# luigifcruz/radio-core

Hardware: AMD Instinct MI355X
Metric: IQ Msamples/s through Tuner+WBFM at 1024 channels (higher is better)
Workload: dtype f32

## Files before the change

### radio-core_amd/csrc/fft_kernel.h

```cpp
#pragma once

#include <hip/hip_runtime.h>

#include <cstdio>
#include <cstdlib>
#include <type_traits>

#include "fft_engine.h"
#include "tile_ns.h"

namespace rcfm {
RCFM_NS_OPEN
namespace fftk {

constexpr int W = RCFM_TILE_W;
constexpr int kLogW = W == 16 ? 4 : W == 8 ? 3 : 2;
static_assert((1 << kLogW) == W, "tile width: 4, 8 or 16 lines");
constexpr int kThreads = 256 * W / 16;

__device__ __forceinline__ float2 cmul(float2 a, float2 b) {
    typedef float v2f __attribute__((ext_vector_type(2)));
    v2f A, B, D;
    A.x = a.x; A.y = a.y; B.x = b.x; B.y = b.y;
    asm("v_pk_mul_f32 %0, %1, %2 op_sel:[0,0] op_sel_hi:[0,1]" : "=v"(D) : "v"(A), "v"(B));
// ... 72 lines not shown
    x0 = cadd(x0, cadd(a, b));
    x1 = cadd_mi(t1, u1);
    x4 = cadd_pi(t1, u1);
    x2 = cadd_mi(t2, u2);
    x3 = cadd_pi(t2, u2);
}

__device__ __forceinline__ void dft7(float2& x0, float2& x1, float2& x2, float2& x3, float2& x4, float2& x5, float2& x6) {
    constexpr float c1 = 0.62348980185873353053f, c2 = -0.22252093395631440429f, c3 = -0.90096886790241912624f;
    constexpr float s1 = 0.78183148246802980871f, s2 = 0.97492791218182360702f, s3 = 0.43388373911755812048f;
    const float2 a1 = cadd(x1, x6), a2 = cadd(x2, x5), a3 = cadd(x3, x4);
    const float2 b1 = csub(x1, x6), b2 = csub(x2, x5), b3 = csub(x3, x4);
    const float2 t1 = make_float2(x0.x + c1 * a1.x + c2 * a2.x + c3 * a3.x, x0.y + c1 * a1.y + c2 * a2.y + c3 * a3.y);
    const float2 t2 = make_float2(x0.x + c2 * a1.x + c3 * a2.x + c1 * a3.x, x0.y + c2 * a1.y + c3 * a2.y + c1 * a3.y);
    const float2 t3 = make_float2(x0.x + c3 * a1.x + c1 * a2.x + c2 * a3.x, x0.y + c3 * a1.y + c1 * a2.y + c2 * a3.y);
    const float2 u1 = make_float2(s1 * b1.x + s2 * b2.x + s3 * b3.x, s1 * b1.y + s2 * b2.y + s3 * b3.y);
    const float2 u2 = make_float2(s2 * b1.x - s3 * b2.x - s1 * b3.x, s2 * b1.y - s3 * b2.y - s1 * b3.y);
    const float2 u3 = make_float2(s3 * b1.x - s1 * b2.x + s2 * b3.x, s3 * b1.y - s1 * b2.y + s2 * b3.y);
    x0 = cadd(x0, cadd(a1, cadd(a2, a3)));
    x1 = cadd_mi(t1, u1);
    x6 = cadd_pi(t1, u1);
    x2 = cadd_mi(t2, u2);
    x5 = cadd_pi(t2, u2);
    x3 = cadd_mi(t3, u3);
    x4 = cadd_pi(t3, u3);
}

template <int R>
__device__ __forceinline__ void dft_nat(float2* v) {
    if constexpr (R == 2) {
        dft2(v[0], v[1]);
    } else if constexpr (R == 3) {
        dft3(v[0], v[1], v[2]);
    } else if constexpr (R == 4) {
        dft4(v[0], v[1], v[2], v[3]);
    } else if constexpr (R == 5) {
        dft5(v[0], v[1], v[2], v[3], v[4]);
    } else if constexpr (R == 7) {
        dft7(v[0], v[1], v[2], v[3], v[4], v[5], v[6]);
    } else {
        constexpr int Ra = (R % 7 == 0) ? 7 : (R % 5 == 0) ? 5 : (R % 4 == 0) ? 4 : (R % 3 == 0) ? 3 : 2;
        constexpr int Rb = R / Ra;
        static_assert(Ra * Rb == R && Rb > 1, "radix must be 2-3-5-7 smooth");
        float2 y[R];
#pragma unroll
        for (int n2 = 0; n2 < Rb; ++n2) {
            float2 t[Ra];
#pragma unroll
            for (int n1 = 0; n1 < Ra; ++n1) t[n1] = v[Rb * n1 + n2];
            dft_nat<Ra>(t);
#pragma unroll
            for (int k1 = 0; k1 < Ra; ++k1) {
                const int m = (n2 * k1) % R;
                if (m == 0) {
                    y[k1 * Rb + n2] = t[k1];
                } else {
                    const double a = -6.28318530717958647692 * (double)m / (double)R;
                    y[k1 * Rb + n2] = cmul(t[k1], make_float2((float)__builtin_cos(a), (float)__builtin_sin(a)));
                }
            }
        }
#pragma unroll
        for (int k1 = 0; k1 < Ra; ++k1) {
            dft_nat<Rb>(&y[k1 * Rb]);
#pragma unroll
            for (int k2 = 0; k2 < Rb; ++k2) v[k1 + Ra * k2] = y[k1 * Rb + k2];
        }
    }
}


__device__ __forceinline__ void dft6(float2* v) {
    dft3(v[0], v[2], v[4]);
    dft3(v[1], v[3], v[5]);
    v[3] = cmul(v[3], make_float2(0.5f, -0.86602540378443864676f));
    v[5] = cmul(v[5], make_float2(-0.5f, -0.86602540378443864676f));
    dft2(v[0], v[1]);
    dft2(v[2], v[3]);
    dft2(v[4], v[5]);
    const float2 y0 = v[0], y3 = v[1], y1 = v[2], y4 = v[3], y2 = v[4], y5 = v[5];
    v[0] = y0; v[1] = y1; v[2] = y2; v[3] = y3; v[4] = y4; v[5] = y5;
}

__device__ __forceinline__ void dft8(float2* v) {
    constexpr float h = 0.70710678118654752440f;
    dft4(v[0], v[2], v[4], v[6]);
    dft4(v[1], v[3], v[5], v[7]);
    v[3] = cmul(v[3], make_float2(h, -h));
    v[5] = mul_mi(v[5]);
    v[7] = cmul(v[7], make_float2(-h, -h));
    dft2(v[0], v[1]);
    dft2(v[2], v[3]);
    dft2(v[4], v[5]);
    dft2(v[6], v[7]);
    const float2 y0 = v[0], y4 = v[1], y1 = v[2], y5 = v[3], y2 = v[4], y6 = v[5], y3 = v[6], y7 = v[7];
    v[0] = y0; v[1] = y1; v[2] = y2; v[3] = y3; v[4] = y4; v[5] = y5; v[6] = y6; v[7] = y7;
}

__device__ __forceinline__ void dft10(float2* v) {
    dft5(v[0], v[2], v[4], v[6], v[8]);
    dft5(v[1], v[3], v[5], v[7], v[9]);
    v[3] = cmul(v[3], make_float2(0.80901699437494742410f, -0.58778525229247312917f));
    v[5] = cmul(v[5], make_float2(0.30901699437494742410f, -0.95105651629515357212f));
    v[7] = cmul(v[7], make_float2(-0.30901699437494742410f, -0.95105651629515357212f));
    v[9] = cmul(v[9], make_float2(-0.80901699437494742410f, -0.58778525229247312917f));
    dft2(v[0], v[1]);
    dft2(v[2], v[3]);
    dft2(v[4], v[5]);
    dft2(v[6], v[7]);
    dft2(v[8], v[9]);
    const float2 y0 = v[0], y5 = v[1], y1 = v[2], y6 = v[3], y2 = v[4], y7 = v[5], y3 = v[6], y8 = v[7],
                 y4 = v[8], y9 = v[9];
    v[0] = y0; v[1] = y1; v[2] = y2; v[3] = y3; v[4] = y4;
    v[5] = y5; v[6] = y6; v[7] = y7; v[8] = y8; v[9] = y9;
}

template <int R>
__device__ __forceinline__ void dif_stage(float2* tile, const float2* tw, int L, int mt, int swz) {
    const int m = mt / R;
    const int step = L / mt;
    const int nb = (L / R) * W;
    for (int e = threadIdx.x; e < nb; e += kThreads) {
        const int w = e & (W - 1);
        const int b = e / W;
        const int g = b / m;
        const int kp = b - g * m;
        const int base = g * mt + kp;
        float2 v[R];
#pragma unroll
        for (int q = 0; q < R; ++q) {
            const int row = base + q * m;
            v[q] = tile[row * W + (w ^ (swz & row & (W - 1)))];
        }
        if constexpr (R == 2) dft2(v[0], v[1]);
        if constexpr (R == 3) dft3(v[0], v[1], v[2]);
        if constexpr (R == 4) dft4(v[0], v[1], v[2], v[3]);
        if constexpr (R == 5) dft5(v[0], v[1], v[2], v[3], v[4]);
        if constexpr (R == 6) dft6(v);
        if constexpr (R == 7) dft7(v[0], v[1], v[2], v[3], v[4], v[5], v[6]);
        if constexpr (R == 8) dft8(v);
        if constexpr (R == 10) dft10(v);
        if constexpr (R > 10) dft_nat<R>(v);
        const int tstep = kp * step;
#pragma unroll
        for (int q = 1; q < R; ++q) v[q] = cmul(v[q], tw[q * tstep]);
#pragma unroll
        for (int q = 0; q < R; ++q) {
            const int row = base + q * m;
            tile[row * W + (w ^ (swz & row & (W - 1)))] = v[q];
        }
    }
}

__device__ __forceinline__ float2 big_twiddle(const FftPassDev& d, unsigned e) {
    const float2 c = d.coarse[e >> d.fine_bits];
    const float th = d.fine_step * (float)(e & ((1u << d.fine_bits) - 1u));
    const float t2 = th * th;
    const float s = th * (1.f - t2 * (1.f / 6.f) * (1.f - t2 * (1.f / 20.f)));
    const float co = 1.f - t2 * 0.5f * (1.f - t2 * (1.f / 12.f) * (1.f - t2 * (1.f / 30.f)));
    return cmul(c, make_float2(co, -s));
}

struct LineId {
    int batch;
    int64_t o1, o2, i;
};

template <class T, class = void>
struct fetch_count { static constexpr int value = 1; };
template <class T>
struct fetch_count<T, std::void_t<decltype(T::kFetches)>> { static constexpr int value = T::kFetches; };

template <class T, class = void>
struct has_ctx : std::false_type {};
template <class T>
struct has_ctx<T, std::void_t<decltype(T::kCtx)>> : std::true_type {};

template <class LoadOp>
__device__ __forceinline__ float2 load_now(const LoadOp& load, const LineId& id, int l, int64_t base, unsigned off) {
    if constexpr (fetch_count<LoadOp>::value == 3)
        return load.post(id, l, load.fetch(id, l, base, off), load.fetch2(id, l, base, off),
                         load.fetch3(id, l, base, off));
    else if constexpr (fetch_count<LoadOp>::value == 2)
        return load.post(id, l, load.fetch(id, l, base, off), load.fetch2(id, l, base, off));
    else if constexpr (has_ctx<LoadOp>::value)
        return load.post(id, l, load.fetch(id, l, base, off), load.prepare(id));
    else
        return load.post(id, l, load.fetch(id, l, base, off));
}

template <class T, class = void>
struct has_half_zones : std::false_type {};
template <class T>
struct has_half_zones<T, std::void_t<decltype(T::kHalfZones)>> : std::bool_constant<T::kHalfZones> {};

template <class T, class = void>
struct has_aux : std::false_type {};
template <class T>
struct has_aux<T, std::void_t<decltype(T::kAux)>> : std::true_type {};

template <class StoreOp>
__device__ __forceinline__ void store_now(const StoreOp& store, const LineId& id, int k, int64_t base, unsigned off,
                                          float2 v) {
    if constexpr (has_aux<StoreOp>::value) store(id, k, base, off, v, store.fetch_aux(id, k, base, off));
    else store(id, k, base, off, v);
}

template <class LoadOp, class StoreOp>
__global__ __launch_bounds__(kThreads) void k_fft_pass(FftPassDev d, LoadOp load, StoreOp store) {
    extern __shared__ __attribute__((aligned(16))) unsigned char smem_raw[];
    const FftPass& p = d.p;
    const int L = p.L;
    float2* tile = reinterpret_cast<float2*>(smem_raw);
    float2* tw = tile + L * W;
    uint16_t* pos = reinterpret_cast<uint16_t*>(tw + L);

    const int tid = threadIdx.x;
    const int64_t tiles_inner = (p.n_inner + W - 1) / W;
    int64_t t = blockIdx.x;
    const int64_t ti = t % tiles_inner;
    t /= tiles_inner;
    LineId id;
    id.batch = blockIdx.y;
    id.o2 = t % p.n_o2;
    id.o1 = t / p.n_o2;
    const int64_t i0 = ti * W;
    const int wvalid = (int)((p.n_inner - i0) < W ? (p.n_inner - i0) : W);
    const int64_t in_base = (int64_t)id.batch * d.in_batch + id.o1 * p.in_o1 + id.o2 * p.in_o2 +
                            (p.in_t ? (i0 >> 4) * p.in_t + (i0 & 15) : i0 * p.in_i);
    const int64_t out_base = (int64_t)id.batch * d.out_batch + id.o1 * p.out_o1 + id.o2 * p.out_o2 +
                             (p.out_t ? (i0 >> 4) * p.out_t + (i0 & 15) : i0 * p.out_i);
    const int swz = p.load_along_l ? (W - 1) : 0;

    for (int e = tid; e < L; e += kThreads) {
        tw[e] = d.stage_tw[e];
        pos[e] = d.pos[e];
    }
    if (p.load_along_l) {
        for (int e = tid; e < L * W; e += kThreads) {
            const int w = e / L, l = e - w * L;
            float2 v = make_float2(0.f, 0.f);
            if (w < wvalid) {
                id.i = i0 + w;
                v = load_now(load, id, l, in_base, (unsigned)(w * p.in_i + l));
            }
            tile[l * W + (w ^ (l & (W - 1)))] = v;
        }
    } else {
        for (int e = tid; e < L * W; e += kThreads) {
            const int l = e / W, w = e & (W - 1);
            float2 v = make_float2(0.f, 0.f);
            if (w < wvalid) {
                id.i = i0 + w;
                v = load_now(load, id, l, in_base, (unsigned)(l * p.in_l + w * p.in_i));
            }
            tile[l * W + w] = v;
        }
    }
    __syncthreads();

    int mt = L;
    for (int s = 0; s < p.nstages; ++s) {
        const int r = p.radix[s];
        switch (r) {
            case 2: dif_stage<2>(tile, tw, L, mt, swz); break;
            case 3: dif_stage<3>(tile, tw, L, mt, swz); break;
            case 4: dif_stage<4>(tile, tw, L, mt, swz); break;
            case 5: dif_stage<5>(tile, tw, L, mt, swz); break;
            case 6: dif_stage<6>(tile, tw, L, mt, swz); break;
            case 7: dif_stage<7>(tile, tw, L, mt, swz); break;
            case 8: dif_stage<8>(tile, tw, L, mt, swz); break;
            case 12: dif_stage<12>(tile, tw, L, mt, swz); break;
            case 15: dif_stage<15>(tile, tw, L, mt, swz); break;
            case 16: dif_stage<16>(tile, tw, L, mt, swz); break;
            case 20: dif_stage<20>(tile, tw, L, mt, swz); break;
            case 24: dif_stage<24>(tile, tw, L, mt, swz); break;
            case 25: dif_stage<25>(tile, tw, L, mt, swz); break;
            case 32: dif_stage<32>(tile, tw, L, mt, swz); break;
            default: dif_stage<10>(tile, tw, L, mt, swz); break;
        }
        mt /= r;
        __syncthreads();
    }

    const unsigned tw_base = (unsigned)(id.o1 * p.tw_o1 + id.o2 * p.tw_o2 + i0 * p.tw_i);
    for (int e = tid; e < L * W; e += kThreads) {
        const int k = e / W, w = e & (W - 1);
        if (w >= wvalid) continue;
        const int row = pos[k];
        float2 v = tile[row * W + (w ^ (swz & row & (W - 1)))];
        if (p.has_twiddle) v = cmul(v, big_twiddle(d, (tw_base + (unsigned)w * (unsigned)p.tw_i) * (unsigned)k));
        id.i = i0 + w;
        store_now(store, id, k, out_base, (unsigned)(k * p.out_k + w * p.out_i), v);
    }
}


constexpr unsigned kXcdGroupMax = 15;
struct BlockPos {
    unsigned tile, batch;
};
struct VBlock {
    unsigned x, y, z, gx, gy, gz;
};
__device__ __forceinline__ VBlock vblock_hw() {
    return VBlock{blockIdx.x, blockIdx.y, blockIdx.z, gridDim.x, gridDim.y, gridDim.z};
}
__device__ __forceinline__ BlockPos block_pos(const VBlock& vb);
__device__ __forceinline__ BlockPos block_pos() { return block_pos(vblock_hw()); }
__device__ __forceinline__ BlockPos block_pos(const VBlock& vb) {
    const unsigned gx = vb.gx, x = vb.x, z = vb.z;
    if (gx <= kXcdGroupMax) {
        if (vb.gy == 1 && (z | 7u) < vb.gz) {
// ... 550 lines not shown
    const bool has1 = c0 + 1 < count;
    const int c1 = has1 ? c0 + 1 : c0;
    const int i0 = (int)bp.tile * W;
    const int left = (int)p1.n_inner - i0;
    const int wvalid = left < W ? left : W;
    const int64_t in_base = (int64_t)id.batch * d1.in_batch + (int64_t)i0 * p1.in_i;
    const int blk16 = mid.blk16;
    const int64_t mid_tile = blk16 ? (int64_t)(i0 >> 4) * blk16 + (i0 & 15) : (int64_t)i0;
    const int64_t mid_base0 = (int64_t)c0 * (blk16 ? mid.stride : d1.out_batch) + mid_tile;
    const int64_t mid_base1 = (int64_t)c1 * (blk16 ? mid.stride : d1.out_batch) + mid_tile;
    const int64_t out_base0 = (int64_t)c0 * d2.out_batch + i0;
    const int64_t out_base1 = (int64_t)c1 * d2.out_batch + i0;
    const unsigned in_i = (unsigned)p1.in_i, mid_k = blk16 ? 16u : (unsigned)p1.out_k, out_k = (unsigned)p2.out_k;
    const int wc = w < wvalid ? w : 0;

    auto lane_off = [&](int it) -> unsigned {
        int g = rg + RG * it;
        if (rowsL % RG != 0) g = g < rowsL ? g : 0;
        return (unsigned)last_stage_base<L, R0, R1, RL, S>(g) * mid_k + (unsigned)wc;
    };
    auto q_off = [&](int q) -> int64_t { return (int64_t)((L / RL) * q) * mid_k; };

    float2 v[nld];
#pragma unroll
    for (int it = 0; it < nld; ++it) {
        int e = tid + T * it;
        if ((L * W) % T != 0) e = e < L * W ? e : 0;
        const int wl = e / L, l = e - wl * L;
        const int wcl = wl < wvalid ? wl : 0;
        id.i = i0 + wcl;
        v[it] = load.fetch(id, l, in_base, (unsigned)wcl * in_i + (unsigned)l);
    }
    for (int e = tid; e < L; e += T) tw[e] = d1.stage_tw[e];
#pragma unroll
    for (int it = 0; it < nld; ++it) {
        const int e = tid + T * it;
        const int wl = e / L, l = e - wl * L;
        id.i = i0 + wl;
        const float2 x = load.post(id, l, v[it]);
        if ((L * W) % T == 0 || e < L * W) tile[lds_slot<true>(l, wl)] = x;
    }
    lds_barrier();
    stage_lds<L, R0, L, true, RG>(tile, tw, w, rg);
    lds_barrier();
    if constexpr (S >= 3) {
        stage_lds<L, R1, L / R0, true, RG>(tile, tw, w, rg);
        lds_barrier();
    }
    if constexpr (S >= 4) {
        stage_lds<L, R2, L / (R0 * R1), true, RG>(tile, tw, w, rg);
        lds_barrier();
    }

    using In0 = decltype(mid.fetch0(mid_base0, mid_base1, 0u));
    In0 a0[nitL * RL];
#pragma unroll
    for (int it = 0; it < nitL; ++it)
#pragma unroll
        for (int q = 0; q < RL; ++q)
            a0[it * RL + q] = mid.fetch0(mid_base0 + q_off(q), mid_base1 + q_off(q), lane_off(it));

    id.i = i0 + w;
    using Keep = typename MidOp::Keep;
    float2 u0[nitL * RL];
    Keep keep[nitL * RL];
#pragma unroll
    for (int it = 0; it < nitL; ++it) {
        const int g = rg + RG * it;
        if ((rowsL % RG == 0) || g < rowsL) {
            float2 x[RL];
#pragma unroll
            for (int q = 0; q < RL; ++q) x[q] = tile[lds_slot<true>(g * RL + q, w)];
            dft_p<RL>(x);
#pragma unroll
            for (int q = 0; q < RL; ++q)
                u0[it * RL + q] = mid.first(x[dft_slot<RL>(q)], a0[it * RL + q], keep[it * RL + q]);
        }
        __builtin_amdgcn_sched_barrier(0);
    }
    lds_barrier();
#pragma unroll
    for (int it = 0; it < nitL; ++it) {
        const int g = rg + RG * it;
        if ((rowsL % RG == 0) || g < rowsL) {
            const int kb = last_stage_base<L, R0, R1, RL, S>(g);
#pragma unroll
            for (int q = 0; q < RL; ++q) tile[lds_slot<true>(kb + (L / RL) * q, w)] = u0[it * RL + q];
        }
    }
    lds_barrier();

    const unsigned f = (unsigned)((int64_t)(i0 + w) * p2.tw_i);
    const float2 D = big_twiddle(d2, f * (unsigned)(L / RL));
    const bool lane_ok = w < wvalid;
    auto second_transform = [&](int64_t out_base) {
        stage_lds<L, R0, L, true, RG>(tile, tw, w, rg);
        lds_barrier();
        if constexpr (S >= 3) {
            stage_lds<L, R1, L / R0, true, RG>(tile, tw, w, rg);
            lds_barrier();
        }
        if constexpr (S >= 4) {
            stage_lds<L, R2, L / (R0 * R1), true, RG>(tile, tw, w, rg);
            lds_barrier();
        }
#pragma unroll
        for (int it = 0; it < nitL; ++it) {
            const int g = rg + RG * it;
            if ((rowsL % RG == 0) || g < rowsL) {
                float2 x[RL];
#pragma unroll
                for (int q = 0; q < RL; ++q) x[q] = tile[lds_slot<true>(g * RL + q, w)];
                dft_p<RL>(x);
                const int kb = last_stage_base<L, R0, R1, RL, S>(g);
                float2 Tw = big_twiddle(d2, f * (unsigned)kb);
                if (lane_ok) {
#pragma unroll
                    for (int q = 0; q < RL; ++q) {
                        const int k = kb + (L / RL) * q;
                        const float2 y = cmul(x[dft_slot<RL>(q)], Tw);
                        Tw = cmul(Tw, D);
                        store(id, k, out_base, (unsigned)k * out_k + (unsigned)w, y);
                    }
                }
            }
        }
    };

    float a1[nitL * RL];
#pragma unroll
    for (int it = 0; it < nitL; ++it)
#pragma unroll
        for (int q = 0; q < RL; ++q) a1[it * RL + q] = mid.fetch1(mid_base1 + q_off(q), lane_off(it));

    second_transform(out_base0);
    if (!has1) return;
    lds_barrier();
#pragma unroll
    for (int it = 0; it < nitL; ++it) {
        const int g = rg + RG * it;
        if ((rowsL % RG == 0) || g < rowsL) {
            const int kb = last_stage_base<L, R0, R1, RL, S>(g);
#pragma unroll
            for (int q = 0; q < RL; ++q) {
                const int k = kb + (L / RL) * q;
                tile[lds_slot<true>(k, w)] = mid.second(keep[it * RL + q], a1[it * RL + q]);
            }
        }
    }
    lds_barrier();
    second_transform(out_base1);
}

template <int L, int R0, int R1, int R2, int R3, int L2, int Q0, int Q1, int T, class LoadOp, class WinOp, class StoreOp>
__global__ __launch_bounds__(T, (T * 16 / W >= 512 ? 4 : 1)) void k_fft_tile2_decim(FftPassDev d1, FftPassDev d2, LoadOp load,
                                                                           WinOp win, StoreOp store) {
    constexpr int S = (R0 > 1) + (R1 > 1) + (R2 > 1) + (R3 > 1);
    static_assert(S >= 2 && R0 * R1 * R2 * R3 == L, "bad radix list");
    static_assert(Q0 * Q1 == L2 && L2 % 2 == 0 && L2 < L, "bad short transform");
    constexpr int RL = (S == 2) ? R1 : (S == 3) ? R2 : R3;
    constexpr int RG = T / W;
    constexpr int nld = (L * W + T - 1) / T;
    constexpr int rowsL = L / RL, nitL = (rowsL + RG - 1) / RG;
    constexpr int nwin = (L2 * W + T - 1) / T;
    __shared__ __attribute__((aligned(16))) float2 tile[L * kRowsPitch];
    __shared__ __attribute__((aligned(16))) float2 tw[L];
    const FftPass& p1 = d1.p;
    const FftPass& p2 = d2.p;
    const int tid = threadIdx.x;
    const int w = tid & (W - 1), rg = tid >> kLogW;

    LineId id;
    const BlockPos bp = block_pos();
    id.batch = bp.batch;
    id.o1 = 0;
    id.o2 = 0;
    const int i0 = (int)bp.tile * W;
    const int left = (int)p1.n_inner - i0;
    const int wvalid = left < W ? left : W;
    const int64_t in_base = (int64_t)id.batch * d1.in_batch + (int64_t)i0 * p1.in_i;
    const int64_t out_base = (int64_t)id.batch * d2.out_batch + i0;
    const unsigned in_i = (unsigned)p1.in_i, out_k = (unsigned)p2.out_k;

    float2 v[nld];
#pragma unroll
    for (int it = 0; it < nld; ++it) {
        int e = tid + T * it;
        if ((L * W) % T != 0) e = e < L * W ? e : 0;
        const int wl = e / L, l = e - wl * L;
        const int wcl = wl < wvalid ? wl : 0;
        id.i = i0 + wcl;
        v[it] = load.fetch(id, l, in_base, (unsigned)wcl * in_i + (unsigned)l);
    }
    float wgt[nwin];
#pragma unroll
    for (int it = 0; it < nwin; ++it) {
        int e = tid + T * it;
        if ((L2 * W) % T != 0) e = e < L2 * W ? e : 0;
        const int wl = e & (W - 1);
        wgt[it] = win.weight(id, e >> kLogW, i0 + (wl < wvalid ? wl : 0));
    }
    for (int e = tid; e < L; e += T) tw[e] = d1.stage_tw[e];
#pragma unroll
    for (int it = 0; it < nld; ++it) {
        const int e = tid + T * it;
        const int wl = e / L, l = e - wl * L;
        id.i = i0 + wl;
        const float2 x = load.post(id, l, v[it]);
        if ((L * W) % T == 0 || e < L * W) tile[lds_slot<true>(l, wl)] = x;
    }
    lds_barrier();
    stage_lds<L, R0, L, true, RG>(tile, tw, w, rg);
    lds_barrier();
    if constexpr (S >= 3) {
        stage_lds<L, R1, L / R0, true, RG>(tile, tw, w, rg);
        lds_barrier();
    }
    if constexpr (S >= 4) {
        stage_lds<L, R2, L / (R0 * R1), true, RG>(tile, tw, w, rg);
        lds_barrier();
    }

    float2 xr[nitL * RL];
#pragma unroll
    for (int it = 0; it < nitL; ++it) {
        const int g = rg + RG * it;
        if ((rowsL % RG == 0) || g < rowsL) {
#pragma unroll
            for (int q = 0; q < RL; ++q) xr[it * RL + q] = tile[lds_slot<true>(g * RL + q, w)];
            dft_p<RL>(&xr[it * RL]);
        }
    }
    lds_barrier();
#pragma unroll
    for (int it = 0; it < nitL; ++it) {
        const int g = rg + RG * it;
        if ((rowsL % RG == 0) || g < rowsL) {
            const int kb = last_stage_base<L, R0, R1, RL, S>(g);
#pragma unroll
            for (int q = 0; q < RL; ++q) {
                if ((L / RL) * q > L2 / 2 && (L / RL) * (q + 1) <= L - L2 / 2) continue;
                const int k = kb + (L / RL) * q;
                int l = -1;
                if (k < L2 / 2) l = k;
                else if (k >= L - L2 / 2) l = k - (L - L2);
                else if (k == L2 / 2) l = L2;
                if (l >= 0) tile[lds_slot<true>(l, w)] = xr[it * RL + dft_slot<RL>(q)];
            }
        }
    }
    for (int e = tid; e < L2; e += T) tw[e] = d2.stage_tw[e];
    lds_barrier();

#pragma unroll
    for (int it = 0; it < nwin; ++it) {
        const int e = tid + T * it;
        if ((L2 * W) % T == 0 || e < L2 * W) {
            const int l = e >> kLogW, wl = e & (W - 1);
            float2 x = tile[lds_slot<true>(l, wl)];
            if (l == L2 / 2 && i0 + wl == 0) {
                const float2 y = tile[lds_slot<true>(L2, wl)];
                x = make_float2(x.x + y.x, x.y + y.y);
            }
            x = make_float2(x.x * wgt[it], x.y * wgt[it]);
            if (l == 0 && i0 + wl == 0) {
                id.i = 0;
                win.dc_bin(id, x);
            }
            tile[lds_slot<true>(l, wl)] = make_float2(x.y, x.x);
        }
    }
    lds_barrier();

    stage_lds<L2, Q0, L2, true, RG>(tile, tw, w, rg);
    lds_barrier();
    constexpr int rows2 = L2 / Q1;
    static_assert(rows2 <= RG, "short transform: one sweep");
    id.i = i0 + w;
    const unsigned f = (unsigned)((int64_t)(i0 + w) * p2.tw_i);
    if (rg < rows2) {
        float2 x[Q1];
#pragma unroll
        for (int q = 0; q < Q1; ++q) x[q] = tile[lds_slot<true>(rg * Q1 + q, w)];
        dft_p<Q1>(x);
        const float2 D = big_twiddle(d2, f * (unsigned)(L2 / Q1));
        float2 Tw = big_twiddle(d2, f * (unsigned)rg);
        if (w < wvalid) {
#pragma unroll
            for (int q = 0; q < Q1; ++q) {
                const int k = rg + (L2 / Q1) * q;
                const float2 y = cmul(x[dft_slot<Q1>(q)], Tw);
                Tw = cmul(Tw, D);
                store(id, k, out_base, (unsigned)k * out_k + (unsigned)w, y);
            }
        }
    }
}


__device__ __forceinline__ float2 stream_load(const float2* p) { return *p; }

__device__ __forceinline__ void stream_store(float2* p, float2 v) {
    if constexpr (W == 16) {
        using v2 = __attribute__((ext_vector_type(2))) float;
        v2 t;
        t.x = v.x;
        t.y = v.y;
        __builtin_nontemporal_store(t, reinterpret_cast<v2*>(p));
    } else {
        *p = v;
    }
}

template <bool SWAP>
struct LoadPlainT {
    const float2* in;
    __device__ __forceinline__ float2 fetch(const LineId&, int, int64_t base, unsigned off) const {
        return stream_load(in + base + off);
    }
    __device__ __forceinline__ float2 post(const LineId&, int, float2 v) const {
        return SWAP ? make_float2(v.y, v.x) : v;
    }
};

template <bool SWAP>
struct StorePlainT {
    float2* out;
    float scale;
    __device__ __forceinline__ void operator()(const LineId&, int, int64_t base, unsigned off, float2 v) const {
        stream_store(out + base + off,
                     SWAP ? make_float2(v.y * scale, v.x * scale) : make_float2(v.x * scale, v.y * scale));
    }
};

struct StoreRowWindow {
    float2* out;
    float scale;
    int n_o1, n_o2, lo, hi;
    int64_t n = 0;
    int halo = 0;
    int sc1_straddle = 0;
    __device__ __forceinline__ void operator()(const LineId& id, int k, int64_t base, unsigned off, float2 v) const {
        const int row = (int)id.o1 + n_o1 * ((int)id.o2 + n_o2 * k);
        const bool keep = lo <= hi ? (row >= lo && row <= hi) : (row >= lo || row <= hi);
        if (!keep) return;
        const float2 y = make_float2(v.x * scale, v.y * scale);
        const int64_t g = base + off;
        const bool straddle = sc1_straddle &&
                              ((reinterpret_cast<uintptr_t>(out + g) - ((uintptr_t)((int)id.i & (W - 1)) << 3)) & 127u) != 0;
        if (straddle) asm volatile("global_store_dwordx2 %0, %1, off sc1" : : "v"(out + g), "v"(y) : "memory");
        else stream_store(out + g, y);
        if (halo > 0) {
            if (g < halo) out[n + g] = y;
            else if (g >= n - halo) out[g - n] = y;
        }
    }
};

}
RCFM_NS_CLOSE
}
namespace rcfm {
RCFM_NS_OPEN
namespace fftk {

#define RCFM_FFT_LONG_TABLE3(X) X(480, 10, 8, 6, 1) X(500, 10, 10, 5, 1)
#define RCFM_FFT_LONG_TABLE(X) X(480, 24, 20, 1, 1) X(500, 25, 20, 1, 1)
#ifndef RCFM_R640
#define RCFM_R640 10, 8, 8, 1
#endif
#ifndef RCFM_R600
#define RCFM_R600 10, 10, 6, 1
#endif
#define RCFM_FFT_BIG_X_(X, LEN, ...) X(LEN, __VA_ARGS__)
#define RCFM_FFT_BIG_LENGTHS(X) RCFM_FFT_BIG_X_(X, 600, RCFM_R600) X(625, 5, 5, 5, 5) RCFM_FFT_BIG_X_(X, 640, RCFM_R640)
#define RCFM_FFT_LENGTHS_(X, LONGT) \
    X(75, 5, 5, 3, 1)            \
    X(80, 10, 8, 1, 1)           \
    X(100, 10, 10, 1, 1)         \
    X(120, 12, 10, 1, 1)         \
    X(125, 5, 5, 5, 1)           \
    X(128, 8, 8, 2, 1)           \
    X(150, 15, 10, 1, 1)         \
    X(160, 16, 10, 1, 1)         \
    X(192, 16, 12, 1, 1)         \
    X(200, 20, 10, 1, 1)         \
    X(240, 24, 10, 1, 1)         \
    X(250, 25, 10, 1, 1)         \
    X(256, 16, 16, 1, 1)         \
    X(300, 20, 15, 1, 1)         \
    X(320, 10, 8, 4, 1)          \
    X(375, 5, 5, 5, 3)           \
    X(384, 8, 8, 6, 1)           \
    X(400, 20, 20, 1, 1)         \
    LONGT(X)                     \
    X(512, 8, 8, 8, 1)
#define RCFM_FFT_FAST_LENGTHS(X) RCFM_FFT_LENGTHS_(X, RCFM_FFT_LONG_TABLE)
#define RCFM_FFT_PAIR_LENGTHS(X) RCFM_FFT_LENGTHS_(X, RCFM_FFT_LONG_TABLE3)


constexpr int tile_threads(int L) {
    return (big_tile_pair(L) ? 1024 : L >= 320 ? 512 : 256) * W / 16;
}

template <class T> struct is_plain_functor : std::false_type {};
template <bool S> struct is_plain_functor<LoadPlainT<S>> : std::true_type {};
template <bool S> struct is_plain_functor<StorePlainT<S>> : std::true_type {};
template <> struct is_plain_functor<StoreRowWindow> : std::true_type {};

enum PassKinds : int { kAnyPass = 0, kStridedOnly = 1, kRowsOnly = 2 };

template <int LEN, int A, int B, int C, int D, bool ROWS, class LoadOp, class StoreOp>
inline void launch_fft_tile_one(const FftPassDev& d, dim3 grid, const LoadOp& ld, const StoreOp& st, hipStream_t s) {
    constexpr int T = tile_threads(LEN);
    hipLaunchKernelGGL((k_fft_tile<LEN, A, B, C, D, ROWS, T, LoadOp, StoreOp>), grid, dim3(T), 0, s, d, ld, st);
}

template <int KIND = kAnyPass, class LoadOp, class StoreOp>
inline void launch_fft_pass(const FftPassDev& d, int batch, const LoadOp& ld, const StoreOp& st, hipStream_t s) {
    bool done = false;
    const bool rows = d.p.load_along_l != 0;
    RC_REQUIRE(!(KIND == kStridedOnly && rows) && !(KIND == kRowsOnly && !rows), RCFM_ERR_RUNTIME,
               "FFT functor used with the wrong pass kind");
    const bool shape_ok = (rows || d.p.in_i == 1) && d.p.out_i == 1 && ((d.p.has_twiddle != 0) == !rows) &&
                          d.p.n_o1 * d.p.n_o2 <= 65535 && batch <= 65535;
    if (shape_ok) {
        const unsigned tiles_inner = (unsigned)((d.p.n_inner + W - 1) / W), outer = (unsigned)(d.p.n_o1 * d.p.n_o2);
        const dim3 grid = d.p.flat_outer ? dim3((tiles_inner * outer + 7u) / 8u * 8u, 1, (unsigned)batch)
                                         : dim3(tiles_inner, outer, (unsigned)batch);
        switch (d.p.L) {
#define RCFM_CASE(LEN, A, B, C, D)                                                                            \
    case LEN:                                                                                                 \
        if (rows) {                                                                                           \
            if constexpr (KIND != kStridedOnly)                                                               \
                launch_fft_tile_one<LEN, A, B, C, D, true, LoadOp, StoreOp>(d, grid, ld, st, s);               \
        } else {                                                                                              \
            if constexpr (KIND != kRowsOnly)                                                                  \
                launch_fft_tile_one<LEN, A, B, C, D, false, LoadOp, StoreOp>(d, grid, ld, st, s);              \
        }                                                                                                     \
        done = true;                                                                                          \
        break;
            RCFM_FFT_FAST_LENGTHS(RCFM_CASE)
            default: break;
        }
        if constexpr (W == 16 && is_plain_functor<LoadOp>::value && is_plain_functor<StoreOp>::value) {
            switch (d.p.L) {
                RCFM_FFT_BIG_LENGTHS(RCFM_CASE)
                default: break;
            }
        }
#undef RCFM_CASE
    }
    if (!done)
        hipLaunchKernelGGL((k_fft_pass<LoadOp, StoreOp>),
                           dim3((unsigned)(d.p.n_o1 * d.p.n_o2 * ((d.p.n_inner + W - 1) / W)), (unsigned)batch, 1),
                           dim3(kThreads), (size_t)d.p.L * (W * sizeof(float2) + sizeof(float2) + sizeof(uint16_t)), s, d,
                           ld, st);
    RC_HIP(hipGetLastError());
}

inline bool fft_tile2_applies(const FftPassDev& d1, const FftPassDev& d2, int batch) {
    bool fast = false;
    switch (d1.p.L) {
#define RCFM_CASE(LEN, A, B, C, D) case LEN:
        RCFM_FFT_FAST_LENGTHS(RCFM_CASE)
#undef RCFM_CASE
        fast = true;
        break;
        default: break;
    }
    return fast && d1.p.load_along_l && !d2.p.load_along_l && d1.p.L == d2.p.L &&
           d1.p.n_inner == d2.p.n_inner && d1.p.n_o1 * d1.p.n_o2 == 1 && d2.p.n_o1 * d2.p.n_o2 == 1 &&
           d1.p.out_k == d2.p.in_l && d2.p.in_i == 1 && d2.p.out_i == 1 && d2.p.has_twiddle && batch <= 65535;
}

#define RCFM_FFT_DECIM_500(X) X(500, 25, 20, 1, 1, 100, 10, 10)
#define RCFM_FFT_DECIM_125(X) X(125, 5, 5, 5, 1, 80, 10, 8)
#define RCFM_FFT_DECIM_PAIRS(X)          \
    RCFM_FFT_DECIM_500(X)                \
    RCFM_FFT_DECIM_125(X)

inline bool fft_tile2_decim_applies(const FftPassDev& d1, const FftPassDev& d2, int batch) {
    bool fast = false;
#define RCFM_CASE(LEN, A, B, C, D, LEN2, E, F) fast = fast || (d1.p.L == LEN && d2.p.L == LEN2);
    RCFM_FFT_DECIM_PAIRS(RCFM_CASE)
#undef RCFM_CASE
    return fast && d1.p.load_along_l && !d2.p.load_along_l &&
           d1.p.n_inner == d2.p.n_inner && d1.p.n_o1 * d1.p.n_o2 == 1 && d2.p.n_o1 * d2.p.n_o2 == 1 &&
           d1.p.out_k == d2.p.in_l && d2.p.in_i == 1 && d2.p.out_i == 1 && d2.p.has_twiddle && batch <= 65535;
}

template <class LoadOp, class WinOp, class StoreOp>
inline bool launch_fft_tile2_decim(const FftPassDev& d1, const FftPassDev& d2, int batch, const LoadOp& ld,
                                   const WinOp& win, const StoreOp& st, hipStream_t s) {
    if (!fft_tile2_decim_applies(d1, d2, batch)) return false;
    const dim3 grid((unsigned)((d1.p.n_inner + W - 1) / W), 1, (unsigned)batch);
    bool done = false;
#define RCFM_CASE(LEN, A, B, C, D, LEN2, E, F)                                                                   \
    if (!done && d1.p.L == LEN && d2.p.L == LEN2) {                                                             \
        hipLaunchKernelGGL((k_fft_tile2_decim<LEN, A, B, C, D, LEN2, E, F, tile_threads(LEN), LoadOp, WinOp, StoreOp>), \
                           grid, dim3(tile_threads(LEN)), 0, s, d1, d2, ld, win, st);                           \
        done = true;                                                                                            \
    }
    RCFM_FFT_DECIM_PAIRS(RCFM_CASE)
#undef RCFM_CASE
    if (!done) return false;
    RC_HIP(hipGetLastError());
    return true;
}

template <class LoadOp, class MidOp, class StoreOp>
inline bool launch_fft_tile2_pair(const FftPassDev& d1, const FftPassDev& d2, int count, const LoadOp& ld,
                                  const MidOp& mid, const StoreOp& st, hipStream_t s) {
    const int pairs = (count + 1) / 2;
    if (!fft_tile2_applies(d1, d2, pairs)) return false;
    const dim3 grid((unsigned)((d1.p.n_inner + W - 1) / W), 1, (unsigned)pairs);
    switch (d1.p.L) {
#define RCFM_CASE(LEN, A, B, C, D)                                                                               \
    case LEN:                                                                                                    \
        hipLaunchKernelGGL((k_fft_tile2_pair<LEN, A, B, C, D, tile_threads(LEN), LoadOp, MidOp, StoreOp>), grid, \
                           dim3(tile_threads(LEN)), 0, s, d1, d2, ld, mid, st, count);                           \
        break;
        RCFM_FFT_PAIR_LENGTHS(RCFM_CASE)
#undef RCFM_CASE
        default: return false;
    }
    RC_HIP(hipGetLastError());
    return true;
}

template <class LoadOp, class MidOp, class StoreOp>
inline bool launch_fft_tile2(const FftPassDev& d1, const FftPassDev& d2, int batch, const LoadOp& ld,
                             const MidOp& mid, const StoreOp& st, hipStream_t s) {
    if (!fft_tile2_applies(d1, d2, batch)) return false;
    const dim3 grid((unsigned)((d1.p.n_inner + W - 1) / W), 1, (unsigned)batch);
    switch (d1.p.L) {
#define RCFM_CASE(LEN, A, B, C, D)                                                                           \
    case LEN:                                                                                                \
        hipLaunchKernelGGL((k_fft_tile2<LEN, A, B, C, D, tile_threads(LEN), LoadOp, MidOp, StoreOp>), grid,  \
                           dim3(tile_threads(LEN)), 0, s, d1, d2, ld, mid, st);                              \
        break;
        RCFM_FFT_FAST_LENGTHS(RCFM_CASE)
#undef RCFM_CASE
        default: return false;
    }
    RC_HIP(hipGetLastError());
    return true;
}

}
RCFM_NS_CLOSE
}
```

Baseline: 34440.

## Fuse decimating FFT bin selection into registers with radix-4 first stage

For the 500→100 decimating FFT pair, the short transform is refactored to a 4×5×5 three-stage factorization. The band-selected bins are kept in registers after the long transform's last radix stage, windowed there, and put straight through a radix-4 butterfly with twiddles. This removes an LDS scatter/gather round trip and one barrier. Coarse twiddle table lookups are hoisted to kernel start to hide their global-load latency. The trade-off is an extra LDS stage for the three-factor short transform and more register pressure.

```diff
diff --git a/radio-core_amd/csrc/fft_kernel.h b/radio-core_amd/csrc/fft_kernel.h
--- a/radio-core_amd/csrc/fft_kernel.h
+++ b/radio-core_amd/csrc/fft_kernel.h
@@ -248,13 +248,18 @@
     }
 }
 
-__device__ __forceinline__ float2 big_twiddle(const FftPassDev& d, unsigned e) {
-    const float2 c = d.coarse[e >> d.fine_bits];
+__device__ __forceinline__ float2 big_twiddle_seed(const FftPassDev& d, unsigned e) {
+    return d.coarse[e >> d.fine_bits];
+}
+__device__ __forceinline__ float2 big_twiddle(const FftPassDev& d, unsigned e, float2 c) {
     const float th = d.fine_step * (float)(e & ((1u << d.fine_bits) - 1u));
     const float t2 = th * th;
     const float s = th * (1.f - t2 * (1.f / 6.f) * (1.f - t2 * (1.f / 20.f)));
     const float co = 1.f - t2 * 0.5f * (1.f - t2 * (1.f / 12.f) * (1.f - t2 * (1.f / 30.f)));
     return cmul(c, make_float2(co, -s));
+}
+__device__ __forceinline__ float2 big_twiddle(const FftPassDev& d, unsigned e) {
+    return big_twiddle(d, e, big_twiddle_seed(d, e));
 }
 
 struct LineId {
@@ -1111,17 +1116,22 @@
     second_transform(out_base1);
 }
 
-template <int L, int R0, int R1, int R2, int R3, int L2, int Q0, int Q1, int T, class LoadOp, class WinOp, class StoreOp>
+template <int L, int R0, int R1, int R2, int R3, int L2, int Q0, int Q1, int Q2, int T, class LoadOp, class WinOp, class StoreOp>
 __global__ __launch_bounds__(T, (T * 16 / W >= 512 ? 4 : 1)) void k_fft_tile2_decim(FftPassDev d1, FftPassDev d2, LoadOp load,
                                                                            WinOp win, StoreOp store) {
     constexpr int S = (R0 > 1) + (R1 > 1) + (R2 > 1) + (R3 > 1);
     static_assert(S >= 2 && R0 * R1 * R2 * R3 == L, "bad radix list");
-    static_assert(Q0 * Q1 == L2 && L2 % 2 == 0 && L2 < L, "bad short transform");
+    constexpr int S2 = (Q0 > 1) + (Q1 > 1) + (Q2 > 1);
+    static_assert(S2 >= 2 && Q0 * Q1 * Q2 == L2 && L2 % 2 == 0 && L2 < L, "bad short transform");
     constexpr int RL = (S == 2) ? R1 : (S == 3) ? R2 : R3;
+    constexpr int QL = (S2 == 2) ? Q1 : Q2;
     constexpr int RG = T / W;
     constexpr int nld = (L * W + T - 1) / T;
     constexpr int rowsL = L / RL, nitL = (rowsL + RG - 1) / RG;
-    constexpr int nwin = (L2 * W + T - 1) / T;
+    constexpr int rows2 = L2 / QL;
+    static_assert(rows2 <= RG, "short transform: one sweep");
+    constexpr bool REG = S == 2 && nitL == 1 && Q0 == 4 && L2 == 4 * rowsL && RL >= 5 && L % L2 == 0;
+    constexpr int nwin = REG ? 4 : (L2 * W + T - 1) / T;
     __shared__ __attribute__((aligned(16))) float2 tile[L * kRowsPitch];
     __shared__ __attribute__((aligned(16))) float2 tw[L];
     const FftPass& p1 = d1.p;
@@ -1152,12 +1162,27 @@
         v[it] = load.fetch(id, l, in_base, (unsigned)wcl * in_i + (unsigned)l);
     }
     float wgt[nwin];
-#pragma unroll
-    for (int it = 0; it < nwin; ++it) {
-        int e = tid + T * it;
-        if ((L2 * W) % T != 0) e = e < L2 * W ? e : 0;
-        const int wl = e & (W - 1);
-        wgt[it] = win.weight(id, e >> kLogW, i0 + (wl < wvalid ? wl : 0));
+    if constexpr (REG) {
+        const int g = rg < rowsL ? rg : 0;
+#pragma unroll
+        for (int q = 0; q < 4; ++q) wgt[q] = win.weight(id, g + rowsL * q, i0 + (w < wvalid ? w : 0));
+    } else {
+#pragma unroll
+        for (int it = 0; it < nwin; ++it) {
+            int e = tid + T * it;
+            if ((L2 * W) % T != 0) e = e < L2 * W ? e : 0;
+            const int wl = e & (W - 1);
+            wgt[it] = win.weight(id, e >> kLogW, i0 + (wl < wvalid ? wl : 0));
+        }
+    }
+    const unsigned f = (unsigned)((int64_t)(i0 + w) * p2.tw_i);
+    const int kb2 = last_stage_base<L2, Q0, Q1, QL, S2>(rg < rows2 ? rg : 0);
+    const float2 seedD = big_twiddle_seed(d2, f * (unsigned)rows2);
+    const float2 seedT = big_twiddle_seed(d2, f * (unsigned)kb2);
+    float2 tw2 = make_float2(0.f, 0.f);
+    if constexpr (REG && S2 == 3) {
+        static_assert(L2 <= T, "short stage table: one entry per thread");
+        tw2 = d2.stage_tw[tid < L2 ? tid : 0];
     }
     for (int e = tid; e < L; e += T) tw[e] = d1.stage_tw[e];
 #pragma unroll
@@ -1190,65 +1215,98 @@
             dft_p<RL>(&xr[it * RL]);
         }
     }
-    lds_barrier();
-#pragma unroll
-    for (int it = 0; it < nitL; ++it) {
-        const int g = rg + RG * it;
-        if ((rowsL % RG == 0) || g < rowsL) {
-            const int kb = last_stage_base<L, R0, R1, RL, S>(g);
-#pragma unroll
-            for (int q = 0; q < RL; ++q) {
-                if ((L / RL) * q > L2 / 2 && (L / RL) * (q + 1) <= L - L2 / 2) continue;
-                const int k = kb + (L / RL) * q;
-                int l = -1;
-                if (k < L2 / 2) l = k;
-                else if (k >= L - L2 / 2) l = k - (L - L2);
-                else if (k == L2 / 2) l = L2;
-                if (l >= 0) tile[lds_slot<true>(l, w)] = xr[it * RL + dft_slot<RL>(q)];
-            }
-        }
-    }
-    for (int e = tid; e < L2; e += T) tw[e] = d2.stage_tw[e];
-    lds_barrier();
-
-#pragma unroll
-    for (int it = 0; it < nwin; ++it) {
-        const int e = tid + T * it;
-        if ((L2 * W) % T == 0 || e < L2 * W) {
-            const int l = e >> kLogW, wl = e & (W - 1);
-            float2 x = tile[lds_slot<true>(l, wl)];
-            if (l == L2 / 2 && i0 + wl == 0) {
-                const float2 y = tile[lds_slot<true>(L2, wl)];
-                x = make_float2(x.x + y.x, x.y + y.y);
-            }
-            x = make_float2(x.x * wgt[it], x.y * wgt[it]);
-            if (l == 0 && i0 + wl == 0) {
+    if constexpr (REG) {
+        float2 y[4];
+        if (rg < rowsL) {
+            y[0] = xr[dft_slot<RL>(0)];
+            y[1] = xr[dft_slot<RL>(1)];
+            y[2] = xr[dft_slot<RL>(RL - 2)];
+            y[3] = xr[dft_slot<RL>(RL - 1)];
+            const bool first = rg == 0 && i0 + w == 0;
+            if (first) y[2] = cadd(y[2], xr[dft_slot<RL>(2)]);
+#pragma unroll
+            for (int q = 0; q < 4; ++q) y[q] = make_float2(y[q].x * wgt[q], y[q].y * wgt[q]);
+            if (first) {
                 id.i = 0;
-                win.dc_bin(id, x);
-            }
-            tile[lds_slot<true>(l, wl)] = make_float2(x.y, x.x);
-        }
-    }
-    lds_barrier();
-
-    stage_lds<L2, Q0, L2, true, RG>(tile, tw, w, rg);
-    lds_barrier();
-    constexpr int rows2 = L2 / Q1;
-    static_assert(rows2 <= RG, "short transform: one sweep");
+                win.dc_bin(id, y[0]);
+            }
+#pragma unroll
+            for (int q = 0; q < 4; ++q) y[q] = make_float2(y[q].y, y[q].x);
+            dft4(y[0], y[1], y[2], y[3]);
+#pragma unroll
+            for (int q = 1; q < 4; ++q) y[q] = cmul(y[q], tw[(L / L2) * q * rg]);
+        }
+        lds_barrier();
+        if (rg < rowsL) {
+#pragma unroll
+            for (int q = 0; q < 4; ++q) tile[lds_slot<true>(rg + rowsL * q, w)] = y[q];
+        }
+        if constexpr (S2 == 3) {
+            if (tid < L2) tw[tid] = tw2;
+        }
+        lds_barrier();
+    } else {
+        lds_barrier();
+#pragma unroll
+        for (int it = 0; it < nitL; ++it) {
+            const int g = rg + RG * it;
+            if ((rowsL % RG == 0) || g < rowsL) {
+                const int kb = last_stage_base<L, R0, R1, RL, S>(g);
+#pragma unroll
+                for (int q = 0; q < RL; ++q) {
+                    if ((L / RL) * q > L2 / 2 && (L / RL) * (q + 1) <= L - L2 / 2) continue;
+                    const int k = kb + (L / RL) * q;
+                    int l = -1;
+                    if (k < L2 / 2) l = k;
+                    else if (k >= L - L2 / 2) l = k - (L - L2);
+                    else if (k == L2 / 2) l = L2;
+                    if (l >= 0) tile[lds_slot<true>(l, w)] = xr[it * RL + dft_slot<RL>(q)];
+                }
+            }
+        }
+        for (int e = tid; e < L2; e += T) tw[e] = d2.stage_tw[e];
+        lds_barrier();
+
+#pragma unroll
+        for (int it = 0; it < nwin; ++it) {
+            const int e = tid + T * it;
+            if ((L2 * W) % T == 0 || e < L2 * W) {
+                const int l = e >> kLogW, wl = e & (W - 1);
+                float2 x = tile[lds_slot<true>(l, wl)];
+                if (l == L2 / 2 && i0 + wl == 0) {
+                    const float2 y = tile[lds_slot<true>(L2, wl)];
+                    x = make_float2(x.x + y.x, x.y + y.y);
+                }
+                x = make_float2(x.x * wgt[it], x.y * wgt[it]);
+                if (l == 0 && i0 + wl == 0) {
+                    id.i = 0;
+                    win.dc_bin(id, x);
+                }
+                tile[lds_slot<true>(l, wl)] = make_float2(x.y, x.x);
+            }
+        }
+        lds_barrier();
+
+        stage_lds<L2, Q0, L2, true, RG>(tile, tw, w, rg);
+        lds_barrier();
+    }
+    if constexpr (S2 == 3) {
+        stage_lds<L2, Q1, L2 / Q0, true, RG>(tile, tw, w, rg);
+        lds_barrier();
+    }
     id.i = i0 + w;
-    const unsigned f = (unsigned)((int64_t)(i0 + w) * p2.tw_i);
     if (rg < rows2) {
-        float2 x[Q1];
-#pragma unroll
-        for (int q = 0; q < Q1; ++q) x[q] = tile[lds_slot<true>(rg * Q1 + q, w)];
-        dft_p<Q1>(x);
-        const float2 D = big_twiddle(d2, f * (unsigned)(L2 / Q1));
-        float2 Tw = big_twiddle(d2, f * (unsigned)rg);
+        float2 x[QL];
+#pragma unroll
+        for (int q = 0; q < QL; ++q) x[q] = tile[lds_slot<true>(rg * QL + q, w)];
+        dft_p<QL>(x);
+        const float2 D = big_twiddle(d2, f * (unsigned)rows2, seedD);
+        float2 Tw = big_twiddle(d2, f * (unsigned)kb2, seedT);
         if (w < wvalid) {
 #pragma unroll
-            for (int q = 0; q < Q1; ++q) {
-                const int k = rg + (L2 / Q1) * q;
-                const float2 y = cmul(x[dft_slot<Q1>(q)], Tw);
+            for (int q = 0; q < QL; ++q) {
+                const int k = kb2 + rows2 * q;
+                const float2 y = cmul(x[dft_slot<QL>(q)], Tw);
                 Tw = cmul(Tw, D);
                 store(id, k, out_base, (unsigned)k * out_k + (unsigned)w, y);
             }
@@ -1433,15 +1491,19 @@
            d1.p.out_k == d2.p.in_l && d2.p.in_i == 1 && d2.p.out_i == 1 && d2.p.has_twiddle && batch <= 65535;
 }
 
-#define RCFM_FFT_DECIM_500(X) X(500, 25, 20, 1, 1, 100, 10, 10)
-#define RCFM_FFT_DECIM_125(X) X(125, 5, 5, 5, 1, 80, 10, 8)
+#ifndef RCFM_DECIM_100
+#define RCFM_DECIM_100 4, 5, 5
+#endif
+#define RCFM_FFT_DECIM_X_(X, ...) X(__VA_ARGS__)
+#define RCFM_FFT_DECIM_500(X) RCFM_FFT_DECIM_X_(X, 500, 25, 20, 1, 1, 100, RCFM_DECIM_100)
+#define RCFM_FFT_DECIM_125(X) X(125, 5, 5, 5, 1, 80, 10, 8, 1)
 #define RCFM_FFT_DECIM_PAIRS(X)          \
     RCFM_FFT_DECIM_500(X)                \
     RCFM_FFT_DECIM_125(X)
 
 inline bool fft_tile2_decim_applies(const FftPassDev& d1, const FftPassDev& d2, int batch) {
     bool fast = false;
-#define RCFM_CASE(LEN, A, B, C, D, LEN2, E, F) fast = fast || (d1.p.L == LEN && d2.p.L == LEN2);
+#define RCFM_CASE(LEN, A, B, C, D, LEN2, E, F, G) fast = fast || (d1.p.L == LEN && d2.p.L == LEN2);
     RCFM_FFT_DECIM_PAIRS(RCFM_CASE)
 #undef RCFM_CASE
     return fast && d1.p.load_along_l && !d2.p.load_along_l &&
@@ -1455,9 +1517,9 @@
     if (!fft_tile2_decim_applies(d1, d2, batch)) return false;
     const dim3 grid((unsigned)((d1.p.n_inner + W - 1) / W), 1, (unsigned)batch);
     bool done = false;
-#define RCFM_CASE(LEN, A, B, C, D, LEN2, E, F)                                                                   \
+#define RCFM_CASE(LEN, A, B, C, D, LEN2, E, F, G)                                                                \
     if (!done && d1.p.L == LEN && d2.p.L == LEN2) {                                                             \
-        hipLaunchKernelGGL((k_fft_tile2_decim<LEN, A, B, C, D, LEN2, E, F, tile_threads(LEN), LoadOp, WinOp, StoreOp>), \
+        hipLaunchKernelGGL((k_fft_tile2_decim<LEN, A, B, C, D, LEN2, E, F, G, tile_threads(LEN), LoadOp, WinOp, StoreOp>), \
                            grid, dim3(tile_threads(LEN)), 0, s, d1, d2, ld, win, st);                           \
         done = true;                                                                                            \
     }
```

After: 34870, median of 6. 1.01x the previous value.
